# datamicroscopes/common

Measured on AMD Instinct MI355X. Metric: score_value evals/sec, higher is better.
Workload: dtype f32

## Files before the change

common_amd/csrc/abi.cpp:

```cpp
#include <algorithm>
#include <atomic>
#include <cmath>
#include <memory>
#include <mutex>
#include <new>

#include "launchers.hpp"

namespace msc {

static thread_local std::string g_last_error;

void set_error(const char *fmt, ...) {
  char buf[1024];
  va_list ap;
  va_start(ap, fmt);
  vsnprintf(buf, sizeof buf, fmt, ap);
  va_end(ap);
  g_last_error = buf;
}
int fail(int code, const char *fmt, ...) {
  char buf[1024];
  va_list ap;
  va_start(ap, fmt);
// ... 1832 lines not shown
      if ((rc = launch(code)) != MSC_OK) break;
      hipError_t e = hipEventRecord(e0, s);
      for (int r = 0; r < 6 && e == hipSuccess; r++) (void)launch(code);
      if (e == hipSuccess) e = hipEventRecord(e1, s);
      if (e == hipSuccess) e = hipEventSynchronize(e1);
      if (e == hipSuccess) e = hipEventElapsedTime(&ms_kind[kind], e0, e1);
      if (e != hipSuccess) rc = fail(MSC_EHIP, "timing failed: %s", hipGetErrorString(e));
    }
    plain_stores = ms_kind[1] < ms_kind[0] ? 1 : 0;
    best = ms_kind[plain_stores];
  }
  (void)hipEventDestroy(e0);
  (void)hipEventDestroy(e1);
  MSC_TRY(rc);
  auto &memo = st->ctx->nich1_shapes;
  for (size_t i = 0; i < memo.size();)
    if (memo[i].out == out_dev && memo[i].nrows == nrows && memo[i].K == st->K) memo.erase(memo.begin() + i);
    else i++;
  memo.insert(memo.begin(), msc_context::ShapeEntry{out_dev, nrows, st->K, shape, plain_stores});
  if (memo.size() > 16) memo.pop_back();
  if (shape_out) *shape_out = shape;
  if (ms_out) *ms_out = best / 6.f;
  return MSC_OK;
}

static int commit(msc_state *st) {
  MSC_TRY(launch_commit_all(st));
  for (auto &h : st->feats) { h.raw_valid = true; h.derived_valid = false; }
  st->crp_valid = false;
  return MSC_OK;
}

enum : uint32_t { kAccZeroed = 0x100, kAccThenPrepare = 0x200 };

static int commit_and_prepare(msc_state *st, bool bump_rng = true) {
  hipStream_t s = st->ctx->stream;
  if (launch_commit_prepare(s, st->desc_dev, (int)st->nfeat, st->K, st->kpad, st->red_i64, st->cnt_u32, st->alpha,
                            st->logpc, bump_rng ? st->rng_dev : nullptr, prepare_value_slices(st)))
    return fail(MSC_EHIP, "k_commit_prepare launch failed");
  for (uint32_t f = 0; f < st->nfeat; f++) {
    const msc_feature_host &h = st->feats[f];
    if (h.family == MSC_NIW && (launch_niw_commit(s, st->desc_dev, f, h.dim, st->K, st->kpad, 1) ||
                                launch_niw_prepare(s, st->desc_dev, f, h.dim, st->K, st->kpad)))
      return fail(MSC_EHIP, "niw commit / prepare launch failed");
    if (h.family == MSC_DM && st->desc_host[f].dm_meta != nullptr &&
        launch_dm_prepare(s, st->desc_dev, (int)f, h.dim, st->kpad, dm_value_slices(h)))
      return fail(MSC_EHIP, "k_dm_prepare launch failed");
  }
  for (auto &h : st->feats) { h.raw_valid = true; h.derived_valid = true; }
  st->crp_valid = true;
  return MSC_OK;
}

static int accumulate_impl(msc_state *st, const msc_dataview *view, const uint32_t *cols, uint64_t row0,
                           uint64_t nrows, const int32_t *z_dev, uint32_t flags) {
  MSC_TRY(bind_view(st, view, cols, row0, nrows));
  hipStream_t s = st->ctx->stream;
  if (flags & MSC_ACC_RESET) {
    if (!(flags & kAccZeroed) && launch_zero64(s, st->red_i64, st->n_i64, st->red_f64, st->n_f64))
      return fail(MSC_EHIP, "k_zero64 launch failed");
  } else {
    MSC_TRY(ensure_raw(st));
    for (uint32_t f = 0; f < st->nfeat; f++)
      if (!st->feats[f].additive_valid) {
        const int rc = st->feats[f].family == MSC_NIW
                           ? launch_niw_commit(s, st->desc_dev, f, st->feats[f].dim, st->K, st->kpad, 0)
                           : launch_lift(s, st->desc_dev + f, 1, st->kpad, st->red_i64, st->cnt_u32, 0);
        if (rc) return fail(MSC_EHIP, "k_lift launch failed");
      }
    if (!st->cnt_additive_valid)
      if (launch_lift(s, st->desc_dev, 0, st->kpad, st->red_i64, st->cnt_u32, 1))
        return fail(MSC_EHIP, "k_lift launch failed");
  }
  for (auto &h : st->feats) h.additive_valid = true;
  st->cnt_additive_valid = true;
  if (nrows > 0) {
    const int rc = launch_accumulate(s, st->ctx->num_cus, st->desc_acc_dev, st->desc_acc_host.data(), (int)st->desc_acc_host.size(),
                                     st->K, st->kpad, row0, nrows, z_dev,
                                     (flags & MSC_ACC_SUBTRACT) ? -1 : 1, st->red_i64);
    if (rc == -2) return fail(MSC_EUNSUPPORTED, "accumulate tables for %u groups exceed LDS", st->K);
    if (rc) return fail(MSC_EHIP, "k_accumulate launch failed: %s", hipGetErrorString(hipGetLastError()));
    for (uint32_t f = 0; f < st->nfeat; f++) {
      if (st->feats[f].family != MSC_NIW) continue;
      MSC_REQUIRE(nrows < (1ull << 32), "niw accumulate takes at most 2^32 - 1 rows per call");
      MSC_HIP(grow_retained(st->retired, st->niw_scratch, 2 * (size_t)st->K + 1 + (size_t)nrows));
      if (launch_niw_accumulate(s, st->ctx->num_cus, st->desc_dev, f, st->K, row0, nrows, z_dev,
                                (flags & MSC_ACC_SUBTRACT) ? -1 : 1, st->niw_scratch, st->feats[f].dim))
        return fail(MSC_EHIP, "niw accumulate launch failed");
    }
  }
  for (auto &h : st->feats) h.raw_valid = false;
  if (flags & kAccThenPrepare) return commit_and_prepare(st);
  if (!(flags & MSC_ACC_NO_COMMIT)) MSC_TRY(commit(st));
  return MSC_OK;
}

extern "C" int msc_accumulate(msc_state *st, const msc_dataview *view, const uint32_t *cols,
                              uint64_t row0, uint64_t nrows, const int32_t *z_dev, uint32_t flags) {
  MSC_REQUIRE(st && (z_dev || nrows == 0), "null argument");
  MSC_REQUIRE((flags & ~(MSC_ACC_RESET | MSC_ACC_SUBTRACT | MSC_ACC_NO_COMMIT)) == 0, "unknown flags 0x%x", flags);
  MSC_HIP(hipSetDevice(st->ctx->device));
  MSC_TRY(device_error_check(st->ctx));
  return accumulate_impl(st, view, cols, row0, nrows, z_dev, flags);
}

extern "C" int msc_entity_op(msc_state *st, const msc_dataview *view, const uint32_t *cols, uint64_t row, uint32_t group,
                             int sign, int32_t *z_dev) {
  MSC_REQUIRE(st && view, "null argument");
  MSC_REQUIRE(sign != 0, "sign must be +1 (join) or -1 (leave)");
  MSC_REQUIRE(group < st->K, "group %u outside [0,%u)", group, st->K);
  MSC_REQUIRE(!st->rng_bump_pending, "msc_entity_op between msc_sweep_step_begin and msc_state_commit_reduce: the additive "
                                     "tables hold uncommitted sums");
  MSC_TRY(device_error_check(st->ctx));
  MSC_HIP(hipSetDevice(st->ctx->device));
  MSC_TRY(bind_view(st, view, cols, row, 1));
  hipStream_t s = st->ctx->stream;
  bool scalar_only = true;
  for (const auto &h : st->feats) scalar_only &= h.family != MSC_NIW && h.family != MSC_DM;
  if (!scalar_only) {
    if (!st->one_z) MSC_TRY(alloc_zeroed(st->one_z, 1));
    if (launch_set_i32(s, st->one_z, (int32_t)group)) return fail(MSC_EHIP, "k_set_i32 launch failed");
    MSC_TRY(accumulate_impl(st, view, cols, row, 1, st->one_z, sign < 0 ? (uint32_t)MSC_ACC_SUBTRACT : 0u));
    if (z_dev && launch_set_i32(s, z_dev + row, sign > 0 ? (int32_t)group : -1)) return fail(MSC_EHIP, "k_set_i32 launch failed");
    return MSC_OK;
  }
  MSC_TRY(ensure_raw(st));
  for (uint32_t f = 0; f < st->nfeat; f++)
    if (!st->feats[f].additive_valid && launch_lift(s, st->desc_dev + f, 1, st->kpad, st->red_i64, st->cnt_u32, 0))
      return fail(MSC_EHIP, "k_lift launch failed");
  if (!st->cnt_additive_valid && launch_lift(s, st->desc_dev, 0, st->kpad, st->red_i64, st->cnt_u32, 1))
    return fail(MSC_EHIP, "k_lift launch failed");
  for (auto &h : st->feats) h.additive_valid = true;
// ... 1265 lines not shown
```

common_amd/csrc/kernels_state.hip:

```cpp
#include "commit_ops.hpp"
#include "device_error.hpp"
#include "family_math.hpp"
#include <cstdarg>
#include <cstdio>
#include "launchers.hpp"

namespace msc {

struct AccShape { uint32_t nu32, nu64, nf64; };
__device__ __host__ inline AccShape acc_shape(int family, uint32_t dim_slice) {
  switch (family) {
    case MSC_BB: return {2, 0, 0};
    case MSC_BBNC: return {2, 0, 0};
    case MSC_GP: return {1, 1, 1};
    case MSC_BNB: return {1, 1, 0};
    case MSC_DM: return {0, dim_slice, 1};
    case MSC_DD: return {dim_slice, 0, 0};
    case MSC_NICH: return {1, 0, 2};
    default: return {0, 0, 0};
  }
}

__global__ __launch_bounds__(1024) void k_accumulate(const FeatDesc *__restrict__ feats, int nfeat,
                                                      uint32_t K, uint32_t kpad, uint64_t row0,
                                                      uint64_t nrows, const int32_t *__restrict__ z,
                                                      int sign, long long *__restrict__ cnt_acc,
                                                      uint32_t dd_slice, uint64_t per) {
  extern __shared__ __attribute__((aligned(16))) unsigned char smem[];
  const uint64_t lo = (uint64_t)blockIdx.y * per;
  const uint64_t hi = lo + per < nrows ? lo + per : nrows;
  if (lo >= hi) return;
  const long long sgn = sign;
  constexpr int U = 8;
  const uint32_t nt = blockDim.x;

  if ((int)blockIdx.x == nfeat) {
    uint32_t *c32 = reinterpret_cast<uint32_t *>(smem);
    for (uint32_t i = threadIdx.x; i < K; i += nt) c32[i] = 0;
    __syncthreads();
    for (uint64_t base = lo; base < hi; base += (uint64_t)U * nt) {
      int g[U];
#pragma unroll
      for (int j = 0; j < U; j++) {
        const uint64_t n = base + threadIdx.x + (uint64_t)j * nt;
        g[j] = n < hi ? z[n] : -1;
      }
#pragma unroll
      for (int j = 0; j < U; j++)
        if ((uint32_t)g[j] < K) atomicAdd(&c32[g[j]], 1u);
    }
    __syncthreads();
    for (uint32_t i = threadIdx.x; i < K; i += nt)
      if (c32[i]) atomicAdd(reinterpret_cast<unsigned long long *>(&cnt_acc[i]),
                            (unsigned long long)(sgn * (long long)c32[i]));
    return;
  }

  const FeatDesc fd = feats[blockIdx.x];
  const bool sliced = fd.family == MSC_DD || fd.family == MSC_DM;
  const uint32_t slice = fd.family == MSC_DM ? (dd_slice > 1 ? dd_slice / 2 : 1) : dd_slice;
  const uint32_t nslices = sliced ? (fd.dim + slice - 1) / slice : 1;
  for (uint32_t sl = 0; sl < nslices; sl++) {
    const uint32_t c_lo = sl * slice;
    const uint32_t c_n = sliced ? (fd.dim - c_lo < slice ? fd.dim - c_lo : slice) : 0;
    const bool fused = fd.fuse_n >= 2;
    const AccShape sh = fused ? AccShape{2u * fd.fuse_n, 0u, 0u} : acc_shape(fd.family, c_n);
    double *f64 = reinterpret_cast<double *>(smem);
    unsigned long long *u64 = reinterpret_cast<unsigned long long *>(f64 + (size_t)K * sh.nf64);
    uint32_t *u32 = reinterpret_cast<uint32_t *>(u64 + (size_t)K * sh.nu64);
    for (uint32_t i = threadIdx.x; i < K * sh.nf64; i += nt) f64[i] = 0.0;
    for (uint32_t i = threadIdx.x; i < K * sh.nu64; i += nt) u64[i] = 0ull;
    for (uint32_t i = threadIdx.x; i < K * sh.nu32; i += nt) u32[i] = 0u;
    __syncthreads();
    const bool scalar_col = fd.family == MSC_BB || fd.family == MSC_BBNC || fd.family == MSC_GP || fd.family == MSC_BNB ||
                            fd.family == MSC_DD || fd.family == MSC_NICH;
    if (scalar_col && fd.mask == nullptr) {
      const bool u8 = fd.family == MSC_BB || fd.family == MSC_BBNC;
      const bool vec4 = hi - lo >= 4 && ((lo | row0) & 3) == 0 && (reinterpret_cast<uintptr_t>(z) & 15) == 0 &&
                        (reinterpret_cast<uintptr_t>(fd.col) & 15) == 0;
      for (uint64_t base = lo; base < hi; base += (uint64_t)U * nt) {
        int g[U];
        uint32_t w[U];
        if (vec4) {
#pragma unroll
          for (int j = 0; j < U / 4; j++) {
            const uint64_t n = base + 4 * ((uint64_t)threadIdx.x + (uint64_t)j * nt);
            const bool whole = n + 3 < hi;
            const uint64_t ns = whole ? n : lo;
            const int4 zq = *reinterpret_cast<const int4 *>(z + ns);
            uint32_t q0, q1, q2, q3;
            if (u8) {
              const uint32_t b = *reinterpret_cast<const uint32_t *>(reinterpret_cast<const uint8_t *>(fd.col) + row0 + ns);
              q0 = b & 0xffu; q1 = (b >> 8) & 0xffu; q2 = (b >> 16) & 0xffu; q3 = b >> 24;
            } else {
              const uint4 b = *reinterpret_cast<const uint4 *>(reinterpret_cast<const uint32_t *>(fd.col) + row0 + ns);
              q0 = b.x; q1 = b.y; q2 = b.z; q3 = b.w;
            }
            g[4 * j] = whole ? zq.x : -1; g[4 * j + 1] = whole ? zq.y : -1; g[4 * j + 2] = whole ? zq.z : -1; g[4 * j + 3] = whole ? zq.w : -1;
            w[4 * j] = q0; w[4 * j + 1] = q1; w[4 * j + 2] = q2; w[4 * j + 3] = q3;
            if (!whole && n < hi) {
#pragma unroll
              for (int c = 0; c < 4; c++) {
                const uint64_t m = n + c;
                if (m < hi) {
                  g[4 * j + c] = z[m];
                  w[4 * j + c] = u8 ? (uint32_t)reinterpret_cast<const uint8_t *>(fd.col)[row0 + m] : reinterpret_cast<const uint32_t *>(fd.col)[row0 + m];
                }
              }
            }
          }
        } else {
#pragma unroll
          for (int j = 0; j < U; j++) {
            const uint64_t n = base + threadIdx.x + (uint64_t)j * nt;
            g[j] = n < hi ? z[n] : -1;
          }
#pragma unroll
          for (int j = 0; j < U; j++) {
            const uint64_t n = base + threadIdx.x + (uint64_t)j * nt;
            const uint64_t row = row0 + (n < hi ? n : lo);
            w[j] = u8 ? (uint32_t)reinterpret_cast<const uint8_t *>(fd.col)[row] : reinterpret_cast<const uint32_t *>(fd.col)[row];
          }
        }
#pragma unroll
        for (int j = 0; j < U; j++) {
          if ((uint32_t)g[j] >= K) continue;
          const uint32_t gg = (uint32_t)g[j], raw = w[j];
          if (fused) {
            uint32_t rest = raw;
// ... 54 lines not shown
        } break;
        case MSC_BNB: {
          const uint32_t v = reinterpret_cast<const uint32_t *>(fd.col)[row];
          atomicAdd(&u32[g], 1u);
          atomicAdd(&u64[g], (unsigned long long)v);
        } break;
        case MSC_DM: {
          const int32_t *x = reinterpret_cast<const int32_t *>(fd.col) + row * fd.dim;
          for (uint32_t i = 0; i < c_n; i++) {
            const uint32_t v = (uint32_t)x[c_lo + i];
            if (v) atomicAdd(&u64[(size_t)i * K + g], (unsigned long long)v);
          }
          if (sl == 0) atomicAdd(&f64[g], dm_row_ratio(fd.dim, x));
        } break;
        case MSC_DD: {
          const int v = reinterpret_cast<const int32_t *>(fd.col)[row];
          if (v >= (int)c_lo && v < (int)(c_lo + c_n)) atomicAdd(&u32[(size_t)(v - c_lo) * K + g], 1u);
        } break;
        case MSC_NICH: {
          const double x = reinterpret_cast<const float *>(fd.col)[row];
          atomicAdd(&u32[g], 1u);
          atomicAdd(&f64[g], x);
          atomicAdd(&f64[K + g], x * x);
        } break;
        default: break;
      }
    }
    __syncthreads();
    for (uint32_t i = threadIdx.x; i < K * sh.nu32; i += nt) {
      const uint32_t r = i / K, k = i - r * K;
      if (!u32[i]) continue;
      uint32_t dst_row = r;
      if (fd.family == MSC_DD) dst_row = c_lo + r;
      const uint32_t mem = r >> 1;
      long long *const mbase = mem == 0 ? fd.fuse_acc[0] : mem == 1 ? fd.fuse_acc[1] : mem == 2 ? fd.fuse_acc[2] : fd.fuse_acc[3];
      long long *dst = fused ? mbase + (size_t)(r & 1u) * kpad + k : &fd.acc_i64[(size_t)dst_row * kpad + k];
      atomicAdd(reinterpret_cast<unsigned long long *>(dst), (unsigned long long)(sgn * (long long)u32[i]));
    }
    for (uint32_t i = threadIdx.x; i < K * sh.nu64; i += nt) {
      const uint32_t r = i / K, k = i - r * K;
      if (!u64[i]) continue;
      const uint32_t dst_row = fd.family == MSC_DM ? c_lo + r : 1 + r;
      atomicAdd(reinterpret_cast<unsigned long long *>(&fd.acc_i64[(size_t)dst_row * kpad + k]),
                (unsigned long long)(sgn * (long long)u64[i]));
    }
    for (uint32_t i = threadIdx.x; i < K * sh.nf64; i += nt) {
      const uint32_t r = i / K, k = i - r * K;
      if (f64[i] != 0.0) atomicAdd(&fd.acc_f64[(size_t)r * kpad + k], (double)sign * f64[i]);
    }
    __syncthreads();
  }
}

MSC_DEV void add_i64(long long *p, long long v) { atomicAdd(reinterpret_cast<unsigned long long *>(p), (unsigned long long)v); }
__global__ __launch_bounds__(256) void k_accumulate_global(const FeatDesc *__restrict__ feats, uint32_t K, uint32_t kpad,
                                                            uint64_t row0, uint64_t nrows, const int32_t *__restrict__ z,
                                                            int sign, long long *__restrict__ cnt_acc) {
  const uint64_t n = (uint64_t)blockIdx.x * 256 + threadIdx.x;
  if (n >= nrows) return;
  const int g = z[n];
  if (g < 0 || (uint32_t)g >= K) return;
  const long long sgn = sign;
  if (blockIdx.y == 0) {
    add_i64(&cnt_acc[g], sgn);
    return;
  }
  const FeatDesc fd = feats[blockIdx.y - 1];
  const uint64_t row = row0 + n;
  if (fd.mask != nullptr) {
    bool m = false;
    if (fd.family == MSC_DM) for (uint32_t e = 0; e < fd.dim; e++) m |= fd.mask[row * fd.dim + e] != 0;
    else m = fd.mask[row] != 0;
    if (m) return;
  }
  switch (fd.family) {
    case MSC_BBNC:
    case MSC_BB:
      add_i64(&fd.acc_i64[(reinterpret_cast<const uint8_t *>(fd.col)[row] != 0 ? 0 : kpad) + g], sgn);
      break;
    case MSC_GP: {
      const uint32_t v = reinterpret_cast<const uint32_t *>(fd.col)[row];
      add_i64(&fd.acc_i64[g], sgn);
      add_i64(&fd.acc_i64[kpad + g], sgn * (long long)v);
      atomicAdd(&fd.acc_f64[g], (double)sign * log_factorial(v));
    } break;
    case MSC_BNB: {
      const uint32_t v = reinterpret_cast<const uint32_t *>(fd.col)[row];
      add_i64(&fd.acc_i64[g], sgn);
      add_i64(&fd.acc_i64[kpad + g], sgn * (long long)v);
    } break;
    case MSC_DM: {
      const int32_t *x = reinterpret_cast<const int32_t *>(fd.col) + row * fd.dim;
      for (uint32_t i = 0; i < fd.dim; i++)
        if (x[i]) add_i64(&fd.acc_i64[(size_t)i * kpad + g], sgn * (long long)(uint32_t)x[i]);
      atomicAdd(&fd.acc_f64[g], (double)sign * dm_row_ratio(fd.dim, x));
    } break;
    case MSC_DD: {
      const int v = reinterpret_cast<const int32_t *>(fd.col)[row];
      if (v >= 0 && v < (int)fd.dim) add_i64(&fd.acc_i64[(size_t)v * kpad + g], sgn);
    } break;
    case MSC_NICH: {
      const double x = reinterpret_cast<const float *>(fd.col)[row];
      add_i64(&fd.acc_i64[g], sgn);
      atomicAdd(&fd.acc_f64[g], (double)sign * x);
      atomicAdd(&fd.acc_f64[kpad + g], (double)sign * x * x);
    } break;
// ... 418 lines not shown
  }
  a.slice_cells = total / shape[dim];
  hipLaunchKernelGGL(k_relation_slice_scores, dim3((unsigned)nent), dim3(256), 0, stream, scores, ld, a, off_dev, ncand, cand_stride,
                     out_dev, ld_out);
  return hipGetLastError() == hipSuccess ? 0 : -1;
}

int launch_relation_blocks(hipStream_t stream, uint32_t ndim, const uint64_t *shape, const int32_t *const *z_dev,
                           const uint32_t *ngroups, const uint32_t *positions_dev, uint64_t ncells, int32_t *out_dev) {
  if (ncells == 0) return 0;
  RelArgs a;
  a.ndim = ndim;
  for (uint32_t d = 0; d < 8; d++) {
    a.shape[d] = d < ndim ? shape[d] : 1;
    a.z[d] = d < ndim ? z_dev[d] : nullptr;
    a.ngroups[d] = d < ndim ? ngroups[d] : 1;
  }
  hipLaunchKernelGGL(k_relation_blocks, dim3((unsigned)((ncells + 255) / 256)), dim3(256), 0, stream, a, positions_dev,
                     ncells, out_dev);
  return hipGetLastError() == hipSuccess ? 0 : -1;
}

int launch_dm_stats(hipStream_t stream, const uint32_t *col, uint64_t n, uint32_t dim, uint32_t *colmax_dev,
                    uint32_t *rowtot_dev) {
  if (n == 0) return 0;
  hipLaunchKernelGGL(k_dm_stats, dim3((unsigned)((n + 255) / 256)), dim3(256), 0, stream, col, n, dim, colmax_dev, rowtot_dev);
  return hipGetLastError() == hipSuccess ? 0 : -1;
}

int launch_col_max_u32(hipStream_t stream, const uint32_t *col, uint64_t n, uint32_t *out_dev) {
  uint64_t blocks = (n + 255) / 256;
  if (blocks > 1024) blocks = 1024;
  if (blocks == 0) blocks = 1;
  hipLaunchKernelGGL(k_col_max_u32, dim3((unsigned)blocks), dim3(256), 0, stream, col, n, out_dev);
  return hipGetLastError() == hipSuccess ? 0 : -1;
}

size_t accumulate_lds_bytes(const FeatDesc *feats_host, int nfeat, uint32_t K, uint32_t dd_slice) {
  size_t need = (size_t)K * 4;
  for (int f = 0; f < nfeat; f++) {
    const uint32_t cap = feats_host[f].family == MSC_DM ? (dd_slice > 1 ? dd_slice / 2 : 1) : dd_slice;
    const uint32_t sl = feats_host[f].family == MSC_DD || feats_host[f].family == MSC_DM
                            ? (feats_host[f].dim < cap ? feats_host[f].dim : cap) : 0;
    AccShape sh = acc_shape(feats_host[f].family, sl);
    if (feats_host[f].fuse_n >= 2) sh = AccShape{2u * feats_host[f].fuse_n, 0u, 0u};
    const size_t b = (size_t)K * (8u * sh.nf64 + 8u * sh.nu64 + 4u * sh.nu32);
    if (b > need) need = b;
  }
  return need;
}

int launch_accumulate(hipStream_t stream, int num_cus, const FeatDesc *feats_dev, const FeatDesc *feats_host,
                      int nfeat, uint32_t K, uint32_t kpad, uint64_t row0, uint64_t nrows,
                      const int32_t *z, int sign, long long *cnt_acc) {
  uint32_t dd_slice = kMaxDDDim;
  while (dd_slice > 1 && (size_t)K * 4u * dd_slice > 64u * 1024u) dd_slice /= 2;
  const size_t lds = accumulate_lds_bytes(feats_host, nfeat, K, dd_slice);
  if (lds > 160u * 1024u) {
    hipLaunchKernelGGL(k_accumulate_global, dim3((unsigned)((nrows + 255) / 256), (unsigned)nfeat + 1), dim3(256), 0, stream,
                       feats_dev, K, kpad, row0, nrows, z, sign, cnt_acc);
    return hipGetLastError() == hipSuccess ? 0 : -1;
  }
  static unsigned long long attr_devices = 0;
  if (first_use_on_device(attr_devices))
    (void)hipFuncSetAttribute(reinterpret_cast<const void *>(k_accumulate),
                              hipFuncAttributeMaxDynamicSharedMemorySize, 160 * 1024);
  constexpr int wgs_per_cu = 8;
  const uint64_t nf1 = (uint64_t)nfeat + 1;
  uint64_t slices = std::max<uint64_t>(1, ((uint64_t)num_cus * wgs_per_cu + nf1 - 1) / nf1);
  uint64_t per = std::max<uint64_t>((nrows + slices - 1) / slices, 4096);
  if ((nrows + per - 1) / per * nf1 < (uint64_t)num_cus)
    per = std::max<uint64_t>(1024, (nrows * nf1 + num_cus - 1) / num_cus);
  slices = std::max<uint64_t>(1, (nrows + per - 1) / per);
  if (slices > 65535) {
    slices = 65535;
    per = (nrows + slices - 1) / slices;
  }
  per = (per + 3) / 4 * 4;
  slices = std::max<uint64_t>(1, (nrows + per - 1) / per);
  const unsigned threads = lds <= 40u * 1024u ? 256u : 1024u;
  hipLaunchKernelGGL(k_accumulate, dim3((unsigned)nf1, (unsigned)slices), dim3(threads), lds, stream, feats_dev, nfeat, K,
                     kpad, row0, nrows, z, sign, cnt_acc, dd_slice, per);
  return hipGetLastError() == hipSuccess ? 0 : -1;
}

int launch_commit(hipStream_t stream, const FeatDesc *feats_dev, int nfeat, uint32_t kpad,
                  const long long *cnt_acc, uint32_t *cnt_u32) {
  hipLaunchKernelGGL(k_commit, dim3((kpad + 255) / 256, nfeat + 1), dim3(256), 0, stream, feats_dev,
                     nfeat, kpad, cnt_acc, cnt_u32);
  return hipGetLastError() == hipSuccess ? 0 : -1;
}

__global__ void k_zero64(unsigned long long *__restrict__ a, size_t na, unsigned long long *__restrict__ b, size_t nb) {
  const size_t stride = (size_t)gridDim.x * blockDim.x;
  for (size_t i = (size_t)blockIdx.x * blockDim.x + threadIdx.x; i < na + nb; i += stride) {
    if (i < na) a[i] = 0ull;
    else b[i - na] = 0ull;
  }
}
__global__ void k_pack64(const long long *__restrict__ i64, size_t ni, const double *__restrict__ f64, size_t nf, double *__restrict__ pack) {
  const size_t stride = (size_t)gridDim.x * blockDim.x;
  for (size_t i = (size_t)blockIdx.x * blockDim.x + threadIdx.x; i < ni + nf; i += stride)
    pack[i] = i < ni ? (double)i64[i] : f64[i - ni];
}
__global__ void k_unpack64(long long *__restrict__ i64, size_t ni, double *__restrict__ f64, size_t nf, const double *__restrict__ pack) {
  const size_t stride = (size_t)gridDim.x * blockDim.x;
  for (size_t i = (size_t)blockIdx.x * blockDim.x + threadIdx.x; i < ni + nf; i += stride) {
    if (i < ni) i64[i] = (long long)pack[i];
    else f64[i - ni] = pack[i];
  }
}
int launch_pack64(hipStream_t stream, bool unpack, long long *i64, size_t ni, double *f64, size_t nf, double *pack) {
  if (ni + nf == 0) return 0;
  const unsigned blocks = (unsigned)std::min<size_t>((ni + nf + 255) / 256, 2048);
  if (unpack) hipLaunchKernelGGL(k_unpack64, dim3(blocks), dim3(256), 0, stream, i64, ni, f64, nf, pack);
  else hipLaunchKernelGGL(k_pack64, dim3(blocks), dim3(256), 0, stream, i64, ni, f64, nf, pack);
  return hipGetLastError() == hipSuccess ? 0 : -1;
}

int launch_zero64(hipStream_t stream, void *a, size_t na, void *b, size_t nb) {
  if (na + nb == 0) return 0;
  const unsigned blocks = (unsigned)std::min<size_t>((na + nb + 255) / 256, 2048);
  hipLaunchKernelGGL(k_zero64, dim3(blocks), dim3(256), 0, stream, static_cast<unsigned long long *>(a), na,
                     static_cast<unsigned long long *>(b), nb);
  return hipGetLastError() == hipSuccess ? 0 : -1;
}

__global__ __launch_bounds__(256) void k_stream_fill(float4 *__restrict__ out, size_t nrows, size_t nslots) {
  const int lane = threadIdx.x & 63;
  const size_t slot = (size_t)blockIdx.x * 4 + (threadIdx.x >> 6);
  if (slot >= nslots) return;
  typedef float f32x4 __attribute__((ext_vector_type(4)));
  const f32x4 zero = {0.f, 0.f, 0.f, 0.f};
  for (size_t rb = slot * 4; rb < nrows; rb += nslots * 4)
#pragma unroll
// ... 41 lines not shown
```

common_amd/csrc/launchers.hpp:

```cpp
#pragma once
#include <algorithm>

#include "msc_internal.hpp"

namespace msc {

inline bool first_use_on_device(unsigned long long &seen) {
  int dev = 0;
  if (hipGetDevice(&dev) != hipSuccess || dev < 0 || dev > 63) return true;
  const unsigned long long bit = 1ull << dev;
  if (seen & bit) return false;
  seen |= bit;
  return true;
}

struct UnpackFeat {
  void *dst;
  uint8_t *dst_mask;
  uint32_t offset;
  uint32_t mask_offset;
  int32_t src_type, dst_type;
  uint32_t count;
  uint32_t pad;
};
// ... 84 lines not shown
#define MSC_NICH_PACK_WAVES 8
#endif
constexpr int kNichPackWaves = MSC_NICH_PACK_WAVES;
#ifndef MSC_NICH_PACK_NC
#define MSC_NICH_PACK_NC 4
#endif
constexpr int kPackMaxLookups = 4;
constexpr int kNichPackNC = MSC_NICH_PACK_NC;
constexpr double kPairTileShare = 0.62;
int launch_sweep_mixed(hipStream_t stream, int num_cus, bool has_dm, ScorePath path, const ScoreShape &shape, const FeatDesc *feats_dev, int nfeat, int nsplit,
                       uint32_t K, uint32_t kpad, uint64_t row0, uint64_t nrows, uint64_t row_id0, int32_t *z,
                       const float *own, const float *crp, const uint64_t *rng, ZeroSpans zero);
int launch_sweep_roles_tail(hipStream_t stream, int num_cus, ScorePath path, const FeatDesc *feats_dev, int nfeat, int nsplit, uint32_t K,
                            uint32_t kpad, uint64_t row0, uint64_t nrows, uint64_t row_id0, int32_t *z, const float *own,
                            const float *crp, const uint64_t *rng, ZeroSpans zero, const float *tail);
int sweep_niw1_max_groups(uint32_t dim);
size_t sweep_nich1_rows_table_floats(uint32_t kpad);
uint32_t sweep_nich1_rows_max_groups();
int launch_sweep_nich1_rows(hipStream_t stream, int num_cus, const FeatDesc *feats_dev, uint32_t K, uint32_t kpad,
                            uint64_t row0, uint64_t nrows, uint64_t row_id0, int32_t *z, const float *crp,
                            const uint64_t *rng, ZeroSpans zero, float *table);
int launch_sweep_niw1(hipStream_t stream, int num_cus, uint32_t dim, const FeatDesc *feats_dev, uint32_t K, uint32_t kpad,
                      uint64_t row0, uint64_t nrows, uint64_t row_id0, int32_t *z, const float *crp, const uint64_t *rng,
                      ZeroSpans zero);
int launch_narrow(hipStream_t stream, int num_cus, int lanes_per_row, uint32_t table_rows, bool sweep, const FeatDesc *feats_dev,
                  int nfeat, uint32_t K, uint32_t kpad, uint64_t row0, uint64_t nrows, const int32_t *z, const float *own,
                  const float *crp, float *out, uint64_t ld, uint64_t row_id0, int32_t *z_out, const uint64_t *rng,
                  ZeroSpans zero);
int launch_sample_rows(hipStream_t stream, int num_cus, const float *scores, uint64_t ld, uint32_t K,
                       uint64_t nrows, uint64_t row_id0, int32_t *z, const uint64_t *rng_dev);
int launch_rng_set(hipStream_t stream, uint64_t *rng_dev, uint64_t seed, uint64_t sweep);
int launch_rng_bump(hipStream_t stream, uint64_t *rng_dev);

constexpr int kSeqThreads = 256;
constexpr uint32_t kSeqMaxGroups = 8192;
constexpr int kSeqMaxFeat = 256;
int launch_sweep_seq(hipStream_t stream, const FeatDesc *feats_dev, int nfeat, uint32_t K, uint32_t kpad, uint64_t row0,
                     uint64_t nrows, uint64_t row_id0, int32_t *z, const uint32_t *order, uint64_t v0, uint64_t v1,
                     uint64_t seed, uint64_t sweep, long long *cnt_acc, uint32_t *cnt_u32, float alpha, float *crp,
                     int32_t *trace);

int launch_niw_prepare(hipStream_t stream, const FeatDesc *feats_dev, uint32_t f, uint32_t dim, uint32_t K,
                       uint32_t kpad);
int launch_niw_score_data(hipStream_t stream, const FeatDesc *feats_dev, uint32_t f, uint32_t K,
                          uint32_t kpad, float *out);
int launch_niw_score(hipStream_t stream, int num_cus, const FeatDesc *feats_dev, uint32_t f, uint32_t dim, uint32_t K,
                     uint32_t kpad, uint64_t row0, uint64_t nrows, const int32_t *z, bool accum, bool f32_fast,
                     double *qown , float *out, uint64_t ld);
int launch_niw_accumulate(hipStream_t stream, int num_cus, const FeatDesc *feats_dev, uint32_t f, uint32_t K,
                          uint64_t row0, uint64_t nrows, const int32_t *z, int sign, uint32_t *scratch_dev, uint32_t dim);
int launch_niw_commit(hipStream_t stream, const FeatDesc *feats_dev, uint32_t f, uint32_t dim, uint32_t K,
                      uint32_t kpad, int to_raw);

int launch_accumulate(hipStream_t stream, int num_cus, const FeatDesc *feats_dev,
                      const FeatDesc *feats_host, int nfeat, uint32_t K, uint32_t kpad, uint64_t row0,
                      uint64_t nrows, const int32_t *z, int sign, long long *cnt_acc);
int launch_commit(hipStream_t stream, const FeatDesc *feats_dev, int nfeat, uint32_t kpad,
                  const long long *cnt_acc, uint32_t *cnt_u32);
int launch_commit_prepare(hipStream_t stream, const FeatDesc *feats_dev, int nfeat, uint32_t K, uint32_t kpad,
                          const long long *cnt_acc, uint32_t *cnt_u32, float alpha, float *crp, uint64_t *rng_bump,
                          uint32_t value_slices);
int launch_pack64(hipStream_t stream, bool unpack, long long *i64, size_t ni, double *f64, size_t nf, double *pack);
int launch_zero64(hipStream_t stream, void *a, size_t na, void *b, size_t nb);
int launch_stream_fill(hipStream_t stream, int num_cus, void *buf, size_t nbytes);
int launch_lift(hipStream_t stream, const FeatDesc *feats_dev, int nfeat, uint32_t kpad,
                long long *cnt_acc, const uint32_t *cnt_u32, int lift_cnt);
int launch_score_data(hipStream_t stream, const FeatDesc *feats_dev, int nfeat, uint32_t K,
                      uint32_t kpad, float *out);
int launch_relation_blocks(hipStream_t stream, uint32_t ndim, const uint64_t *shape, const int32_t *const *z_dev,
                           const uint32_t *ngroups, const uint32_t *positions_dev, uint64_t ncells, int32_t *out_dev);
int launch_relation_slice_scores(hipStream_t stream, const float *scores, uint64_t ld, uint32_t ndim, const uint64_t *shape,
                                 uint32_t dim, const uint32_t *seg_dev, const uint32_t *ids_dev, const int32_t *off_dev,
                                 uint32_t ncand, uint32_t cand_stride, uint64_t nent, float *out_dev, uint64_t ld_out);
int launch_dm_stats(hipStream_t stream, const uint32_t *col, uint64_t n, uint32_t dim, uint32_t *colmax_dev,
                    uint32_t *rowtot_dev);
int launch_col_max_u32(hipStream_t stream, const uint32_t *col, uint64_t n, uint32_t *out_dev);
int launch_mask_sentinel(hipStream_t stream, const void *col, const uint8_t *mask, uint64_t n, bool bytes, uint32_t sentinel, void *out);
int launch_pack_bits(hipStream_t stream, const void *const *cols, int m, uint32_t radix, uint64_t n, void *out);
int launch_pack_nich_x(hipStream_t stream, const float *const *cols_dev, uint32_t n2, uint32_t n2p, uint64_t n, float *out);
int launch_pack_look_idx(hipStream_t stream, const LookIdxSrc *src_dev, uint32_t nsrc, uint32_t l4, uint64_t n, uint32_t *out);
int launch_fuse_tables(hipStream_t stream, const FeatDesc *feats_dev, int nsplit, int nblocks, uint32_t kpad);
int launch_hp_grid_score(hipStream_t stream, const HpJob *jobs_dev, uint32_t njobs, uint32_t max_points, uint32_t K,
                         uint32_t kpad, const uint32_t *cnt, const uint8_t *slots, uint32_t nblk, double *part,
                         double *out);
int launch_crp_grid_score(hipStream_t stream, const HpJob *job_dev, uint32_t npoints, const uint32_t *cnt, uint32_t K,
                          double *out);
int launch_hp_grid_draw(hipStream_t stream, const HpJob *jobs_dev, uint32_t njobs, const double *scores, uint64_t seed,
                        uint64_t sweep, uint32_t *chosen);
int launch_hp_slice(hipStream_t stream, const SliceTarget *targets_dev, uint32_t ntargets, const SliceCoord *coords_dev,
                    uint32_t K, uint32_t kpad, const uint32_t *cnt, const uint8_t *slots, uint64_t key, uint64_t sweep,
                    float *values, uint32_t *evals, uint32_t *status);
inline uint32_t theta_slice_blocks(uint32_t K) { return (K + 255) / 256; }
int launch_theta_slice(hipStream_t stream, const ThetaJob *jobs_dev, uint32_t njobs, uint32_t K, uint32_t kpad,
                       const uint32_t *cnt, const uint8_t *slots, uint64_t key, uint64_t sweep,
                       unsigned long long *evals_part, uint32_t *bad_part);
int launch_unpack(hipStream_t stream, const uint8_t *records, const uint8_t *mask, uint64_t nrows,
                  uint32_t rowsize, uint32_t maskrowsize, const void *feats_dev, uint32_t nfeat);

int launch_pred_prepare(hipStream_t stream, const PredFeat *pfs_dev, const std::vector<PredFeat> &pfs, uint32_t K,
                        uint32_t kpad);
int launch_pred_sample(hipStream_t stream, const PredFeat *pfs_dev, const std::vector<PredFeat> &pfs, uint32_t K,
                       uint64_t row0, uint64_t nrows, uint64_t row_id0, const int32_t *z, int32_t *z_out,
                       bool masked_only, uint64_t seed, uint64_t sweep);

int launch_marginal_norm(hipStream_t stream, const uint32_t *cnt, uint32_t K, float alpha, double *norm);
int launch_marginal_nich1(hipStream_t stream, int num_cus, const FeatDesc *feats_dev, uint32_t K, uint32_t kpad, uint64_t row0,
                          uint64_t nrows, const int32_t *z, const float *crp, const double *norm, float *logp, int32_t *map,
                          float *logresp);
int launch_marginal_tile(hipStream_t stream, int num_cus, const FeatDesc *feats_dev, int nfeat, int nsplit, uint32_t K,
// ... 20 lines not shown
```

common_amd/csrc/msc_internal.hpp:

```cpp
#pragma once

#include <hip/hip_runtime.h>

#include <cstdarg>
#include <cstdint>
#include <cstdio>
#include <cstring>
#include <string>
#include <vector>

#include "../../include/microscopes_hip.h"
#include "dev_buf.hpp"

namespace msc {

constexpr int kWave = 64;
constexpr int kGroupTile = 256;
constexpr unsigned kMaxDDDim = 128;
constexpr int kGrpRows = 128;
constexpr unsigned kGpMaxTable = 1024;
constexpr float kNtFastGbps = 6650.f;

void set_error(const char *fmt, ...);
int fail(int code, const char *fmt, ...);
// ... 372 lines not shown
  msc::DevBuf<msc::FeatDesc> desc_dev;
  std::vector<msc::FeatDesc> desc_host;
  msc::DevBuf<msc::FeatDesc> desc_tile_dev;
  std::vector<msc::FeatDesc> desc_tile_host;
  uint32_t tile_split = 0;
  msc::DevBuf<msc::FeatDesc> desc_fuse_dev;
  std::vector<msc::FeatDesc> desc_fuse_host;
  uint32_t fuse_nfeat = 0, fuse_split = 0;
  bool fuse_any = false;
  msc::DevBuf<float> fuse_tab;
  msc::DevBuf<msc::FeatDesc> desc_acc_dev;
  std::vector<msc::FeatDesc> desc_acc_host;
  msc::DevBuf<msc::NichPlanInfo> nich_info;
  msc::DevBuf<float> rn_pack;
  msc::DevBuf<msc::NichPos> rn_pos;
  bool nich_blocks_any = false;
  const msc_dataview *bound_view = nullptr;
  uint64_t bound_serial = 0;
  std::vector<uint32_t> bound_cols;
  msc::Retired retired;
  msc::DevBuf<float> scratch;
  msc::DevBuf<float> tail_scores;
  msc::DevBuf<float> own;
  msc::ScorePath tile_path = msc::MSC_PATH_TILE;
  msc::PlanCost plan_cost;
  bool tile_narrow_tail_ok = false;
  uint32_t tail_max_rows = 0, tail_pack_rows = 0;
  bool tail_masked_nich = false;
  bool tail_dm = false;
  msc::DevBuf<float> tail_pack;
  uint32_t loo_staged = 0;
  msc::DevBuf<double> marg_norm;
  msc::DevBuf<float> rows_table;
  msc::DevBuf<uint32_t> colmax_dev;
  msc::DevBuf<uint64_t> rng_dev;
  uint64_t rng_seed = 0, rng_sweep = 0;
  bool rng_valid = false;
  bool rng_bump_pending = false;
  uint64_t rng_next_sweep = 0;
  struct StepGraph {
    hipGraphExec_t exec = nullptr;
    const void *view = nullptr, *z = nullptr;
    uint64_t view_serial = 0, row0 = 0, nrows = 0, row_id0 = 0;
    float alpha = 0.f;
    std::vector<uint32_t> cols;
    std::vector<uint8_t> flags;
    int seen = 0;
    bool disabled = false;
    uint64_t n_eager = 0, n_replayed = 0;
  } step_graph;
  msc::DevBuf<double> niw_qown;
  msc::DevBuf<int32_t> one_z;
  msc::DevBuf<uint32_t> niw_scratch;
  std::vector<std::unique_ptr<msc_hp_grid>> hp_grids;
  msc::DevBuf<double> hp_part;
  msc::DevBuf<double> hp_out;
  msc::DevBuf<msc::HpJob> hp_jobs_dev;
  msc::DevBuf<uint32_t> hp_chosen_dev;
  std::vector<msc::HpJob> hp_jobs_host;
  msc::DevBuf<unsigned char> slice_buf;
  msc::DevBuf<msc::PredFeat> pred_feats_dev;
  msc::DevBuf<double> pred_par;
  msc::DevBuf<int32_t> pred_z;
  std::vector<msc::PredFeat> pred_feats_host;
  msc::PinnedBuf<msc::PredFeat> pred_stage;
  hipEvent_t pred_upload = nullptr;
  bool pred_upload_pending = false;
};

struct msc_zmatrix {
  msc_context *ctx = nullptr;
  uint64_t n = 0;
  uint32_t m = 0, nlabels = 0, nt = 0;
  bool wide = false;
  msc::DevBuf<uint32_t> rows_dev;
  msc::DevBuf<uint32_t> order_dev;
  msc::DevBuf<uint32_t> batch;
  msc::DevBuf<uint32_t> bad;
  msc::DevBuf<uint32_t> counts;
  uint32_t staged = 0;
  uint64_t nsamples = 0;
};
```

Measured before the change: 1729 billion.

## Bucket rows by group before accumulate to merge run-length LDS atomics

Adds a pre-pass kernel that counting-sorts each 4096-row tile by group id into an order buffer. The accumulate kernel then walks the sorted order per thread, collapsing consecutive same-group rows into one LDS atomic per run for scalar families. It is meant to cut LDS atomic contention, at the cost of an extra kernel, an order buffer, gathered column reads, and extra LDS for a staging array. The workload metric is score_value, which may not run accumulate at all.

```diff
diff --git a/common_amd/csrc/abi.cpp b/common_amd/csrc/abi.cpp
--- a/common_amd/csrc/abi.cpp
+++ b/common_amd/csrc/abi.cpp
@@ -1908,6 +1908,15 @@
   return MSC_OK;
 }
 
+static bool route_accumulate(const msc_state *st) {
+  if (st->K > kBucketMaxGroups || st->desc_acc_host.size() < 2) return false;
+  for (const FeatDesc &d : st->desc_acc_host) {
+    const bool runs = d.family == MSC_BB || d.family == MSC_BBNC || d.family == MSC_GP || d.family == MSC_BNB || d.family == MSC_NICH;
+    if (runs && d.mask == nullptr) return true;
+  }
+  return false;
+}
+
 static int accumulate_impl(msc_state *st, const msc_dataview *view, const uint32_t *cols, uint64_t row0,
                            uint64_t nrows, const int32_t *z_dev, uint32_t flags) {
   MSC_TRY(bind_view(st, view, cols, row0, nrows));
@@ -1931,9 +1940,14 @@
   for (auto &h : st->feats) h.additive_valid = true;
   st->cnt_additive_valid = true;
   if (nrows > 0) {
+    uint32_t *order = nullptr;
+    if (route_accumulate(st)) {
+      MSC_HIP(grow_retained(st->retired, st->acc_order, accumulate_order_words(nrows)));
+      order = st->acc_order;
+    }
     const int rc = launch_accumulate(s, st->ctx->num_cus, st->desc_acc_dev, st->desc_acc_host.data(), (int)st->desc_acc_host.size(),
                                      st->K, st->kpad, row0, nrows, z_dev,
-                                     (flags & MSC_ACC_SUBTRACT) ? -1 : 1, st->red_i64);
+                                     (flags & MSC_ACC_SUBTRACT) ? -1 : 1, st->red_i64, order);
     if (rc == -2) return fail(MSC_EUNSUPPORTED, "accumulate tables for %u groups exceed LDS", st->K);
     if (rc) return fail(MSC_EHIP, "k_accumulate launch failed: %s", hipGetErrorString(hipGetLastError()));
     for (uint32_t f = 0; f < st->nfeat; f++) {
diff --git a/common_amd/csrc/kernels_state.hip b/common_amd/csrc/kernels_state.hip
--- a/common_amd/csrc/kernels_state.hip
+++ b/common_amd/csrc/kernels_state.hip
@@ -25,7 +25,8 @@
                                                       uint32_t K, uint32_t kpad, uint64_t row0,
                                                       uint64_t nrows, const int32_t *__restrict__ z,
                                                       int sign, long long *__restrict__ cnt_acc,
-                                                      uint32_t dd_slice, uint64_t per) {
+                                                      uint32_t dd_slice, uint64_t per,
+                                                      const uint32_t *__restrict__ order, uint32_t vals_off) {
   extern __shared__ __attribute__((aligned(16))) unsigned char smem[];
   const uint64_t lo = (uint64_t)blockIdx.y * per;
   const uint64_t hi = lo + per < nrows ? lo + per : nrows;
@@ -74,7 +75,87 @@
     __syncthreads();
     const bool scalar_col = fd.family == MSC_BB || fd.family == MSC_BBNC || fd.family == MSC_GP || fd.family == MSC_BNB ||
                             fd.family == MSC_DD || fd.family == MSC_NICH;
-    if (scalar_col && fd.mask == nullptr) {
+    if (order != nullptr && scalar_col && fd.mask == nullptr && fd.family != MSC_DD) {
+      uint32_t *vals = reinterpret_cast<uint32_t *>(smem + vals_off);
+      const bool u8 = fd.family == MSC_BB || fd.family == MSC_BBNC;
+      const uint32_t P = kBucketRows / nt;
+      for (uint64_t s0 = lo; s0 < hi; s0 += kBucketRows) {
+        const uint32_t cnt = (uint32_t)(hi - s0 < kBucketRows ? hi - s0 : kBucketRows);
+        const uint4 *mine = reinterpret_cast<const uint4 *>(order + s0 + (uint64_t)threadIdx.x * P);
+        uint4 e4 = mine[0];
+        for (uint32_t i = threadIdx.x; i < cnt; i += nt) {
+          const uint64_t row = row0 + s0 + i;
+          vals[i] = u8 ? (uint32_t)reinterpret_cast<const uint8_t *>(fd.col)[row] : reinterpret_cast<const uint32_t *>(fd.col)[row];
+        }
+        __syncthreads();
+        uint32_t cur = 0xffffffffu, n = 0, c[8] = {0, 0, 0, 0, 0, 0, 0, 0};
+        unsigned long long su = 0ull;
+        double da = 0.0, db = 0.0;
+        auto flush_run = [&]() {
+          if (n == 0) return;
+          if (fused) {
+#pragma unroll
+            for (uint32_t m = 0; m < 8; m++)
+              if (c[m]) atomicAdd(&u32[(size_t)m * K + cur], c[m]);
+          } else if (u8) {
+            if (c[0]) atomicAdd(&u32[cur], c[0]);
+            if (c[1]) atomicAdd(&u32[K + cur], c[1]);
+          } else {
+            atomicAdd(&u32[cur], n);
+            if (fd.family == MSC_NICH) {
+              atomicAdd(&f64[cur], da);
+              atomicAdd(&f64[K + cur], db);
+            } else {
+              atomicAdd(&u64[cur], su);
+              if (fd.family == MSC_GP) atomicAdd(&f64[cur], da);
+            }
+          }
+          n = 0;
+          su = 0ull;
+          da = db = 0.0;
+#pragma unroll
+          for (uint32_t m = 0; m < 8; m++) c[m] = 0;
+        };
+        for (uint32_t q = 0; q < P; q += 4) {
+          const uint32_t e[4] = {e4.x, e4.y, e4.z, e4.w};
+          if (q + 4 < P) e4 = mine[q / 4 + 1];
+#pragma unroll
+          for (int j = 0; j < 4; j++) {
+            const uint32_t gg = e[j] >> 16, at = e[j] & 0xffffu;
+            if (gg >= K || at >= cnt) continue;
+            if (gg != cur) {
+              flush_run();
+              cur = gg;
+            }
+            const uint32_t raw = vals[at];
+            n++;
+            if (fused) {
+              uint32_t rest = raw;
+#pragma unroll
+              for (uint32_t m = 0; m < 4; m++) {
+                if (m >= fd.fuse_n) break;
+                const uint32_t d = fd.fuse_radix == 2 ? (rest & 1u) : rest % 3u;
+                rest = fd.fuse_radix == 2 ? rest >> 1 : rest / 3u;
+                c[2 * m] += d == 1u ? 1u : 0u;
+                c[2 * m + 1] += d == 0u ? 1u : 0u;
+              }
+            } else if (u8) {
+              c[0] += raw != 0 ? 1u : 0u;
+              c[1] += raw != 0 ? 0u : 1u;
+            } else if (fd.family == MSC_NICH) {
+              const double x = __uint_as_float(raw);
+              da += x;
+              db += x * x;
+            } else {
+              su += raw;
+              if (fd.family == MSC_GP) da += log_factorial(raw);
+            }
+          }
+        }
+        flush_run();
+        __syncthreads();
+      }
+    } else if (scalar_col && fd.mask == nullptr) {
       const bool u8 = fd.family == MSC_BB || fd.family == MSC_BBNC;
       const bool vec4 = hi - lo >= 4 && ((lo | row0) & 3) == 0 && (reinterpret_cast<uintptr_t>(z) & 15) == 0 &&
                         (reinterpret_cast<uintptr_t>(fd.col) & 15) == 0;
@@ -235,6 +316,60 @@
   }
 }
 
+__global__ __launch_bounds__(1024) void k_bucket_rows(const int32_t *__restrict__ z, uint64_t nrows, uint32_t K,
+                                                       uint32_t *__restrict__ order) {
+  static_assert(kBucketRows == 4096 && kBucketMaxGroups == 4096, "four rows and four groups a thread");
+  __shared__ uint32_t cnt[kBucketMaxGroups];
+  __shared__ uint32_t sorted[kBucketRows];
+  __shared__ uint32_t wsum[16];
+  const uint32_t tid = threadIdx.x, lane = tid & 63u, wave = tid >> 6;
+  const uint64_t base = (uint64_t)blockIdx.x * kBucketRows;
+#pragma unroll
+  for (int j = 0; j < 4; j++) cnt[tid + j * 1024u] = 0u;
+  __syncthreads();
+  int g[4];
+  uint32_t rank[4];
+#pragma unroll
+  for (int j = 0; j < 4; j++) {
+    const uint64_t n = base + tid + (uint64_t)j * 1024u;
+    const int gg = n < nrows ? z[n] : -1;
+    g[j] = (uint32_t)gg < K ? gg : -1;
+  }
+#pragma unroll
+  for (int j = 0; j < 4; j++) rank[j] = g[j] >= 0 ? atomicAdd(&cnt[g[j]], 1u) : 0u;
+  __syncthreads();
+  const uint32_t c0 = cnt[4 * tid], c1 = cnt[4 * tid + 1], c2 = cnt[4 * tid + 2], c3 = cnt[4 * tid + 3];
+  const uint32_t own = c0 + c1 + c2 + c3;
+  uint32_t incl = own;
+#pragma unroll
+  for (int off = 1; off < 64; off <<= 1) {
+    const uint32_t o = (uint32_t)__shfl_up((int)incl, off, 64);
+    if ((int)lane >= off) incl += o;
+  }
+  if (lane == 63u) wsum[wave] = incl;
+  __syncthreads();
+  uint32_t before = 0u, total = 0u;
+  for (uint32_t w = 0; w < 16u; w++) {
+    before += w < wave ? wsum[w] : 0u;
+    total += wsum[w];
+  }
+  const uint32_t excl = before + incl - own;
+  cnt[4 * tid] = excl;
+  cnt[4 * tid + 1] = excl + c0;
+  cnt[4 * tid + 2] = excl + c0 + c1;
+  cnt[4 * tid + 3] = excl + c0 + c1 + c2;
+  __syncthreads();
+#pragma unroll
+  for (int j = 0; j < 4; j++)
+    if (g[j] >= 0) sorted[cnt[g[j]] + rank[j]] = ((uint32_t)g[j] << 16) | (tid + (uint32_t)j * 1024u);
+  __syncthreads();
+#pragma unroll
+  for (int j = 0; j < 4; j++) {
+    const uint32_t p = tid + (uint32_t)j * 1024u;
+    order[base + p] = p < total ? sorted[p] : kBucketFiller;
+  }
+}
+
 MSC_DEV void add_i64(long long *p, long long v) { atomicAdd(reinterpret_cast<unsigned long long *>(p), (unsigned long long)v); }
 __global__ __launch_bounds__(256) void k_accumulate_global(const FeatDesc *__restrict__ feats, uint32_t K, uint32_t kpad,
                                                             uint64_t row0, uint64_t nrows, const int32_t *__restrict__ z,
@@ -759,10 +894,17 @@
 
 int launch_accumulate(hipStream_t stream, int num_cus, const FeatDesc *feats_dev, const FeatDesc *feats_host,
                       int nfeat, uint32_t K, uint32_t kpad, uint64_t row0, uint64_t nrows,
-                      const int32_t *z, int sign, long long *cnt_acc) {
+                      const int32_t *z, int sign, long long *cnt_acc, uint32_t *order) {
   uint32_t dd_slice = kMaxDDDim;
   while (dd_slice > 1 && (size_t)K * 4u * dd_slice > 64u * 1024u) dd_slice /= 2;
-  const size_t lds = accumulate_lds_bytes(feats_host, nfeat, K, dd_slice);
+  size_t lds = accumulate_lds_bytes(feats_host, nfeat, K, dd_slice);
+  const uint32_t vals_off = (uint32_t)((lds + 15) & ~(size_t)15);
+  if (order != nullptr) {
+    if (K > kBucketMaxGroups || vals_off + kBucketRows * 4u > 160u * 1024u) return -1;
+    lds = vals_off + kBucketRows * 4u;
+    hipLaunchKernelGGL(k_bucket_rows, dim3((unsigned)((nrows + kBucketRows - 1) / kBucketRows)), dim3(1024), 0, stream, z, nrows, K, order);
+    if (hipGetLastError() != hipSuccess) return -1;
+  }
   if (lds > 160u * 1024u) {
     hipLaunchKernelGGL(k_accumulate_global, dim3((unsigned)((nrows + 255) / 256), (unsigned)nfeat + 1), dim3(256), 0, stream,
                        feats_dev, K, kpad, row0, nrows, z, sign, cnt_acc);
@@ -784,10 +926,11 @@
     per = (nrows + slices - 1) / slices;
   }
   per = (per + 3) / 4 * 4;
+  if (order != nullptr) per = (per + kBucketRows - 1) / kBucketRows * kBucketRows;
   slices = std::max<uint64_t>(1, (nrows + per - 1) / per);
-  const unsigned threads = lds <= 40u * 1024u ? 256u : 1024u;
+  const unsigned threads = (order != nullptr ? (size_t)vals_off : lds) <= 40u * 1024u ? 256u : 1024u;
   hipLaunchKernelGGL(k_accumulate, dim3((unsigned)nf1, (unsigned)slices), dim3(threads), lds, stream, feats_dev, nfeat, K,
-                     kpad, row0, nrows, z, sign, cnt_acc, dd_slice, per);
+                     kpad, row0, nrows, z, sign, cnt_acc, dd_slice, per, order, vals_off);
   return hipGetLastError() == hipSuccess ? 0 : -1;
 }
 
diff --git a/common_amd/csrc/launchers.hpp b/common_amd/csrc/launchers.hpp
--- a/common_amd/csrc/launchers.hpp
+++ b/common_amd/csrc/launchers.hpp
@@ -160,9 +160,11 @@
 int launch_niw_commit(hipStream_t stream, const FeatDesc *feats_dev, uint32_t f, uint32_t dim, uint32_t K,
                       uint32_t kpad, int to_raw);
 
+constexpr uint32_t kBucketRows = 4096, kBucketMaxGroups = 4096, kBucketFiller = 0xffffffffu;
+inline size_t accumulate_order_words(uint64_t nrows) { return (size_t)((nrows + kBucketRows - 1) / kBucketRows) * kBucketRows; }
 int launch_accumulate(hipStream_t stream, int num_cus, const FeatDesc *feats_dev,
                       const FeatDesc *feats_host, int nfeat, uint32_t K, uint32_t kpad, uint64_t row0,
-                      uint64_t nrows, const int32_t *z, int sign, long long *cnt_acc);
+                      uint64_t nrows, const int32_t *z, int sign, long long *cnt_acc, uint32_t *order);
 int launch_commit(hipStream_t stream, const FeatDesc *feats_dev, int nfeat, uint32_t kpad,
                   const long long *cnt_acc, uint32_t *cnt_u32);
 int launch_commit_prepare(hipStream_t stream, const FeatDesc *feats_dev, int nfeat, uint32_t K, uint32_t kpad,
diff --git a/common_amd/csrc/msc_internal.hpp b/common_amd/csrc/msc_internal.hpp
--- a/common_amd/csrc/msc_internal.hpp
+++ b/common_amd/csrc/msc_internal.hpp
@@ -448,6 +448,7 @@
   msc::DevBuf<double> niw_qown;
   msc::DevBuf<int32_t> one_z;
   msc::DevBuf<uint32_t> niw_scratch;
+  msc::DevBuf<uint32_t> acc_order;
   std::vector<std::unique_ptr<msc_hp_grid>> hp_grids;
   msc::DevBuf<double> hp_part;
   msc::DevBuf<double> hp_out;
```

Measured after the change: 1668 billion. 0.965x the previous value.
